# TorbenHellriegel/Speaker-Recognition-x-vectors

Measured on AMD Instinct MI355X. Metric: x-vector embeddings/sec (300-frame utt), higher is better.
Workload: dtype f32; 1 GPU; configs[1]: 1xMI355X batch=256 fixed 300-frame x 24-MFCC utterances, fp32 frame-level stack, extract_x_vec layer 6, random-init weights seed 42; build=xvec_hip gfx950 build df48636768b7, batch_per_gpu=256, frames=300

## Files before the change

### speaker-recognition-x-vectors_amd/csrc/tdnn_common.h

```cpp
#pragma once
#include "xvec_internal.h"

namespace xvec {

typedef float f32x16 __attribute__((ext_vector_type(16)));
typedef unsigned int u32x4 __attribute__((ext_vector_type(4)));
typedef float f32x4 __attribute__((ext_vector_type(4)));
typedef __bf16 bf16x8 __attribute__((ext_vector_type(8)));

#define SB() __builtin_amdgcn_sched_barrier(0)

__device__ __forceinline__ int xcd_remap(int bid, int nwg) {
    const int q = nwg >> 3, r = nwg & 7, xcd = bid & 7, local = bid >> 3;
    const int base = (xcd < r) ? xcd * (q + 1) : r * (q + 1) + (xcd - r) * q;
    return base + local;
}

typedef float f32x2 __attribute__((ext_vector_type(2)));
typedef __bf16 bf16x2 __attribute__((ext_vector_type(2)));

__device__ __forceinline__ float add_halves(float x) {
    const unsigned u = __float_as_uint(x);
    const auto r = __builtin_amdgcn_permlane32_swap(u, u, false, false);
    return __uint_as_float(r[0]) + __uint_as_float(r[1]);
}

__device__ __forceinline__ unsigned long long uniform64(unsigned long long v) {
    const unsigned lo = __builtin_amdgcn_readfirstlane((unsigned)v);
    const unsigned hi = __builtin_amdgcn_readfirstlane((unsigned)(v >> 32));
    return ((unsigned long long)hi << 32) | lo;
}

__device__ __forceinline__ __amdgpu_buffer_rsrc_t make_rsrc_n(const void* p, int num_bytes) {
    void* q = reinterpret_cast<void*>(uniform64(reinterpret_cast<unsigned long long>(p)));
    return __builtin_amdgcn_make_buffer_rsrc(q, (short)0, __builtin_amdgcn_readfirstlane(num_bytes), 0x00020000);
}

__device__ __forceinline__ __amdgpu_buffer_rsrc_t make_rsrc(const void* p) { return make_rsrc_n(p, 0x7fffffff); }

__device__ __forceinline__ __amdgpu_buffer_rsrc_t make_rsrc_bounded(const void* base, int64_t off, int64_t total) {
    int64_t left = total - off;
    left = left < 0 ? 0 : (left > 0x7fffffff ? 0x7fffffff : left);
    return make_rsrc_n(static_cast<const char*>(base) + off, (int)left);
}

__device__ __forceinline__ float4 buf_load16(__amdgpu_buffer_rsrc_t rsrc, int voff, int soff) {
    const u32x4 v = __builtin_amdgcn_raw_buffer_load_b128(rsrc, voff, soff, 0);
    const f32x4 f = __builtin_bit_cast(f32x4, v);
    return make_float4(f.x, f.y, f.z, f.w);
}

__device__ __forceinline__ void group_range(const TdnnArgs& a, int p, int64_t& begin, int64_t& end) {
    int64_t g_begin, g_end;
    if (a.pair_period > 0) {
        const int P = a.blocks_per_col, PQ = a.pair_period, hq = PQ >> 1;
        const int64_t base = a.groups_total / P;
        const int rem = (int)(a.groups_total % P);
        const int rem1 = rem < (P >> 1) ? rem : (P >> 1), rem2 = rem - rem1;
        const int xq = p / PQ, w = p % PQ;
        const int nf = xq * hq + (w < hq ? w : hq);
        const int ns = xq * hq + (w > hq ? w - hq : 0);
        g_begin = base * p + (nf < rem1 ? nf : rem1) + (ns < rem2 ? ns : rem2);
        const bool extra = (w < hq) ? (nf < rem1) : (ns < rem2);
        g_end = g_begin + base + (extra ? 1 : 0);
    } else {
        g_begin = a.groups_total * (int64_t)p / a.blocks_per_col;
        g_end = a.groups_total * (int64_t)(p + 1) / a.blocks_per_col;
    }
    begin = g_begin;
    end = g_end;
}

__host__ __device__ __forceinline__ int wino_pair_count(int T, int d) {
    const int r = T % (2 * d);
    return d * (T / (2 * d)) + (r < d ? r : d);
}

typedef unsigned u32x2 __attribute__((ext_vector_type(2)));

__device__ __forceinline__ void split3(const float4& v, u32x2& hi, u32x2& mid, u32x2& lo) {
    typedef __bf16 bf16x4v __attribute__((ext_vector_type(4)));
    const f32x4 x = {v.x, v.y, v.z, v.w};
    const bf16x4v h = __builtin_convertvector(x, bf16x4v);
    const f32x4 r1 = x - __builtin_convertvector(h, f32x4);
    const bf16x4v m = __builtin_convertvector(r1, bf16x4v);
    const f32x4 r2 = r1 - __builtin_convertvector(m, f32x4);
    const bf16x4v l = __builtin_convertvector(r2, bf16x4v);
    hi = __builtin_bit_cast(u32x2, h);
    mid = __builtin_bit_cast(u32x2, m);
    lo = __builtin_bit_cast(u32x2, l);
}

__device__ __forceinline__ void s3_mfma6(f32x16& acc, const float4* x, const float4* w) {
#define XV_S3M(xp_, wp_) \
    acc = __builtin_amdgcn_mfma_f32_32x32x16_bf16(__builtin_bit_cast(bf16x8, x[xp_]), __builtin_bit_cast(bf16x8, w[wp_]), acc, 0, 0, 0);
    XV_S3M(2, 0) XV_S3M(1, 1) XV_S3M(0, 2) XV_S3M(1, 0) XV_S3M(0, 1) XV_S3M(0, 0)
#undef XV_S3M
}

__device__ __forceinline__ void store_acc(const f32x16& v, const float4 (&sc)[4], const float4 (&sh)[4],
                                          __amdgpu_buffer_rsrc_t yrsrc, int y_voff, int y_soff) {
    unsigned pk[8];
    typedef float f32x2v __attribute__((ext_vector_type(2)));
#pragma unroll
    for (int gq = 0; gq < 4; ++gq) {
        const float y0 = fmaf(fmaxf(v[4 * gq + 0], 0.f), sc[gq].x, sh[gq].x);
        const float y1 = fmaf(fmaxf(v[4 * gq + 1], 0.f), sc[gq].y, sh[gq].y);
        const float y2 = fmaf(fmaxf(v[4 * gq + 2], 0.f), sc[gq].z, sh[gq].z);
        const float y3 = fmaf(fmaxf(v[4 * gq + 3], 0.f), sc[gq].w, sh[gq].w);
        pk[2 * gq] = __builtin_bit_cast(unsigned, __builtin_convertvector(f32x2v{y0, y1}, bf16x2));
        pk[2 * gq + 1] = __builtin_bit_cast(unsigned, __builtin_convertvector(f32x2v{y2, y3}, bf16x2));
    }
#pragma unroll
    for (int pr = 0; pr < 2; ++pr) {
        auto r0 = __builtin_amdgcn_permlane32_swap(pk[4 * pr + 0], pk[4 * pr + 2], false, false);
        auto r1 = __builtin_amdgcn_permlane32_swap(pk[4 * pr + 1], pk[4 * pr + 3], false, false);
        const u32x4 o = {r0[0], r1[0], r0[1], r1[1]};
        __builtin_amdgcn_raw_buffer_store_b128(o, yrsrc, y_voff, y_soff + pr * 32, 0);
        asm volatile("s_nop 1" ::"v"(o));
    }
}

__device__ __forceinline__ float lower_half(float x) {
    const unsigned u = __float_as_uint(x);
    const auto r = __builtin_amdgcn_permlane32_swap(u, u, false, false);
    return __uint_as_float(r[0]);
}

constexpr int kPoolPlanes = 3;

__device__ __forceinline__ void store_partial(__amdgpu_buffer_rsrc_t prs, int ld, int64_t slot, int h, int col, float k,
                                              float v0, float v1) {
    const int soff = (int)(slot * kPoolPlanes * ld) * 4;
    __builtin_amdgcn_raw_buffer_store_b32(__float_as_uint(h ? v1 : v0), prs, (col + (1 + h) * ld) * 4, soff, 0);
    if (h == 0) __builtin_amdgcn_raw_buffer_store_b32(__float_as_uint(k), prs, col * 4, soff, 0);
}

__device__ __forceinline__ void store_partial2(__amdgpu_buffer_rsrc_t prs, int ld, int64_t slot, int h, int col, float ka,
                                               float kb, float s1a, float s2a, float s1b, float s2b) {
    typedef unsigned u32x2 __attribute__((ext_vector_type(2)));
    const int soff = (int)(slot * kPoolPlanes * ld) * 4;
    const u32x2 v = {__float_as_uint(h ? s2a : s1a), __float_as_uint(h ? s2b : s1b)};
    __builtin_amdgcn_raw_buffer_store_b64(v, prs, (col + (1 + h) * ld) * 4, soff, 0);
    if (h == 0) {
        const u32x2 kv = {__float_as_uint(ka), __float_as_uint(kb)};
        __builtin_amdgcn_raw_buffer_store_b64(kv, prs, col * 4, soff, 0);
    }
}

struct PoolCur {
    int u;
    int64_t end;
};

__device__ __forceinline__ int64_t sload_i64(const int64_t* p) {
    int64_t v;
    asm volatile("s_load_dwordx2 %0, %1, 0x0\n\ts_waitcnt lgkmcnt(0)" : "=s"(v) : "s"(p) : "memory");
    return v;
}

template <bool RAGGED>
__device__ __forceinline__ int64_t first_row(const RowMap& m, int u) {
    u = __builtin_amdgcn_readfirstlane(u);
    if (RAGGED) return sload_i64(m.offsets + u) - (int64_t)u * m.cum;
    return (int64_t)u * (m.fixed_T - m.cum);
}

__device__ __forceinline__ float max1(float x, float m) {
    float r;
    asm("v_max_f32 %0, %1, %2" : "=v"(r) : "v"(x), "v"(m));
    return r;
}

template <bool RAGGED>
__device__ __forceinline__ void pool_group_impl(const TdnnArgs& a, const f32x16& v, float negk, int64_t row_g, int h,
                                                int col, PoolCur& pc) {
    const int64_t grp = row_g >> 5;
    const RowMap& m = a.out_map;
    const __amdgpu_buffer_rsrc_t prs = make_rsrc(a.pool_part);
    while (pc.end <= row_g && pc.u < m.n_utts - 1) {
        pc.u = __builtin_amdgcn_readfirstlane(pc.u + 1);
        pc.end = first_row<RAGGED>(m, pc.u + 1);
    }
    const float K = -negk;
    if (pc.end >= row_g + 32) {
        float a0 = max1(v[0], negk), a1 = max1(v[1], negk), a2 = max1(v[2], negk), a3 = max1(v[3], negk);
        float b0 = a0 * a0, b1 = a1 * a1, b2 = a2 * a2, b3 = a3 * a3;
#pragma unroll
        for (int e = 4; e < 16; e += 4) {
            const float d0 = max1(v[e], negk), d1 = max1(v[e + 1], negk), d2 = max1(v[e + 2], negk), d3 = max1(v[e + 3], negk);
            a0 += d0; a1 += d1; a2 += d2; a3 += d3;
            b0 = fmaf(d0, d0, b0); b1 = fmaf(d1, d1, b1); b2 = fmaf(d2, d2, b2); b3 = fmaf(d3, d3, b3);
        }
        const float s1 = add_halves((a0 + a1) + (a2 + a3)), s2 = add_halves((b0 + b1) + (b2 + b3));
        store_partial(prs, a.ldy, grp + pc.u, h, col, K, s1, s2);
        return;
    }
    for (int u = pc.u; u < m.n_utts; u = __builtin_amdgcn_readfirstlane(u + 1)) {
        const int64_t off = first_row<RAGGED>(m, u);
        if (off >= row_g + 32) break;
        const int64_t end = first_row<RAGGED>(m, u + 1);
        const int64_t lo_r = off > row_g ? off : row_g;
        const int64_t hi_r = end < row_g + 32 ? end : row_g + 32;
        if (hi_r <= lo_r) continue;
        const int lo_l = (int)(lo_r - row_g), hi_l = (int)(hi_r - row_g);
        const unsigned below_hi = hi_l >= 32 ? 0xffffffffu : ((1u << hi_l) - 1u);
        const unsigned rowmask = below_hi & ~((1u << lo_l) - 1u);
        const unsigned lm = rowmask >> (4 * h);
        float s1 = 0.f, s2 = 0.f;
#pragma unroll
        for (int e = 0; e < 16; ++e) {
            const float d = ((lm >> ((e & 3) + 8 * (e >> 2))) & 1u) ? max1(v[e], negk) : 0.f;
            s1 += d;
            s2 = fmaf(d, d, s2);
        }
        s1 = add_halves(s1);
        s2 = add_halves(s2);
        store_partial(prs, a.ldy, grp + u, h, col, K, s1, s2);
    }
}

__device__ __forceinline__ void pool_group(const TdnnArgs& a, const f32x16& v, float negk, int64_t row_g, int h, int col,
                                           PoolCur& pc) {
    if (a.out_map.offsets == nullptr) pool_group_impl<false>(a, v, negk, row_g, h, col, pc);
    else pool_group_impl<true>(a, v, negk, row_g, h, col, pc);
}

__device__ __forceinline__ PoolCur pool_cursor(const TdnnArgs& a, int64_t row) {
    PoolCur pc;
    pc.u = __builtin_amdgcn_readfirstlane(utt_of_row(a.out_map, row));
    pc.end = row_off(a.out_map, pc.u + 1);
    return pc;
}

}
```

### speaker-recognition-x-vectors_amd/csrc/tdnn_layer_impl.h

```cpp
#pragma once
#include <cstdlib>

#include "tdnn_common.h"

namespace xvec {

constexpr int kBM = 128, kBN = 128;
constexpr int kStageFloats = (kBM + kBN) * kBK;
constexpr int kConstFloats = 3 * kBN;
constexpr int kLdsBytes = (2 * kStageFloats + kConstFloats) * 4;

#ifdef XVEC_DIAG
static __device__ unsigned long long g_diag[8 * 8192];
#endif

struct Ctx {
    __amdgpu_buffer_rsrc_t xrsrc;
    __amdgpu_buffer_rsrc_t wrsrc;
    int x_base;
    int ur0, ur1, ur2, ur3;
    int xo0, xo1, xo2, xo3;
    int w_toff;
    __amdgpu_buffer_rsrc_t wfrsrc;
    int wf_voff;
    int r0;
    int u_tile;
    int64_t off_next;
    int64_t m0;
    int64_t g_s, g_end;
    PoolCur pool;
    bool pivot_set;
    int tap, kc, itl;
    int es;
};

__device__ __forceinline__ float4 cvt8_bf16(const float4& lo, const float4& hi) {
    typedef __bf16 bf16x8v __attribute__((ext_vector_type(8)));
    typedef float f32x8v __attribute__((ext_vector_type(8)));
    const f32x8v f8 = {lo.x, lo.y, lo.z, lo.w, hi.x, hi.y, hi.z, hi.w};
    const f32x4 b4 = __builtin_bit_cast(f32x4, __builtin_convertvector(f8, bf16x8v));
    return make_float4(b4.x, b4.y, b4.z, b4.w);
}

template <bool RAGGED>
__device__ __forceinline__ void set_tile_rows_impl(const TdnnArgs& a, Ctx& cx) {
    const int n_last = a.out_map.n_utts - 1;
    const int64_t t_out = a.out_map.fixed_T - a.out_map.cum;
    auto next_off = [&](int u) -> int64_t {
        if (RAGGED) return a.out_map.offsets[u + 1] - (int64_t)(u + 1) * a.out_map.cum;
        return (int64_t)(u + 1) * t_out;
    };
    while (cx.m0 >= cx.off_next && cx.u_tile < n_last) {
        cx.u_tile = __builtin_amdgcn_readfirstlane(cx.u_tile + 1);
        cx.off_next = next_off(cx.u_tile);
    }
    const int64_t p = cx.m0 + cx.r0;
    int c0 = 0, c1 = 0, c2 = 0, c3 = 0;
    int u = cx.u_tile;
    int64_t nxt = cx.off_next;
    while (nxt < cx.m0 + 128 && u < n_last) {
        c0 += (p >= nxt) ? 1 : 0;
        c1 += (p + 32 >= nxt) ? 1 : 0;
        c2 += (p + 64 >= nxt) ? 1 : 0;
        c3 += (p + 96 >= nxt) ? 1 : 0;
        u = __builtin_amdgcn_readfirstlane(u + 1);
        nxt = next_off(u);
    }
    const int rb = a.ldx * cx.es;
    cx.ur0 = (cx.u_tile + c0) * a.span;
    cx.ur1 = (cx.u_tile + c1) * a.span;
    cx.ur2 = (cx.u_tile + c2) * a.span;
    cx.ur3 = (cx.u_tile + c3) * a.span;
    cx.xo0 = cx.x_base + cx.ur0 * rb;
    cx.xo1 = cx.x_base + cx.ur1 * rb;
    cx.xo2 = cx.x_base + cx.ur2 * rb;
    cx.xo3 = cx.x_base + cx.ur3 * rb;
}

__device__ __forceinline__ void set_tile_rows(const TdnnArgs& a, Ctx& cx) {
    if (a.span == 0) {
        cx.ur0 = cx.ur1 = cx.ur2 = cx.ur3 = 0;
        cx.xo0 = cx.xo1 = cx.xo2 = cx.xo3 = cx.x_base;
        return;
    }
    if (a.out_map.offsets == nullptr) set_tile_rows_impl<false>(a, cx);
    else set_tile_rows_impl<true>(a, cx);
}

template <int GUARD>
__device__ __forceinline__ __amdgpu_buffer_rsrc_t x_rsrc(const TdnnArgs& a, const Ctx& cx) {
    const int src_es = GUARD == 2 ? 4 : cx.es;
    const int64_t off = cx.m0 * (int64_t)a.ldx * src_es;
    if (GUARD) return make_rsrc_bounded(a.X, off, a.x_bytes ? a.x_bytes : a.x_rows * (int64_t)a.ldx * src_es);
    return make_rsrc(static_cast<const char*>(a.X) + off);
}

template <int GUARD, bool X3>
__device__ __forceinline__ void advance(const TdnnArgs& a, Ctx& cx, int n_chunks) {
    if (cx.itl + 1 < n_chunks) {
        ++cx.itl;
        if (++cx.tap == a.n_taps) {
            cx.tap = 0;
            ++cx.kc;
        }
    } else {
        const int64_t g_rem = cx.g_end - cx.g_s;
        const int64_t g_next = cx.g_s + (g_rem < 4 ? g_rem : 4);
        if (g_next < cx.g_end) {
            cx.g_s = g_next;
            cx.m0 = g_next * 32;
            cx.xrsrc = x_rsrc<GUARD>(a, cx);
            set_tile_rows(a, cx);
            cx.itl = 0;
            cx.kc = 0;
            cx.tap = 0;
        }
    }
}

#define XV_KO(q_) ((((2 * (q_)) + h) ^ sw) << 2)
#define XV_FRG_A(i_, q_, f_, S_) \
    if constexpr (G > i_) { rg.fa##i_##_##f_ = *reinterpret_cast<const float4*>((S_) + a_rd + i_ * 32 * kBK + XV_KO(q_)); }
#define XV_FRG_B(q_, f_, S_) \
    if constexpr (!INBF) { rg.fb_##f_ = *reinterpret_cast<const float4*>((S_) + b_rd + XV_KO(q_)); }
#define XV_LST_A(i_, n_) \
    if constexpr (G > i_) { *reinterpret_cast<float4*>(smem + n_ * kStageFloats + st_off + i_ * 32 * kBK) = rg.sA##i_##_##n_; }
#define XV_LST_B(j_, n_)                                                                                  \
    if constexpr (X3) {                                                                                   \
        if constexpr (G > j_) *reinterpret_cast<float4*>(smem + n_ * kStageFloats + st_off + kBM * kBK + j_ * 32 * kBK) = rg.sB##j_##_##n_; \
    } else if constexpr (!INBF) {                                                                         \
        *reinterpret_cast<float4*>(smem + n_ * kStageFloats + st_off + kBM * kBK + j_ * 32 * kBK) = rg.sB##j_##_##n_; \
    }
#define XV_LST3(i_, b_)                                                                                   \
    if constexpr (G > i_) {                                                                               \
        *reinterpret_cast<float4*>(smem + b_ * kStageFloats + st_off + i_ * 32 * kBK) = rg.sA##i_##_0;      \
        *reinterpret_cast<float4*>(smem + b_ * kStageFloats + st_off + kBM * kBK + i_ * 32 * kBK) = rg.sB##i_##_0; \
    }
#define XV_GLD_X(dst_, i_, P_OFF)                                                                         \
    {                                                                                                     \
        const int row_shift = cx.tap * a.tap_rows;                                                        \
        const int soff = ((row_shift + 32 * i_) * a.ldx + cx.kc * BKE) * ES + (P_OFF);                    \
        if (GUARD) {                                                                                      \
                  \
            const bool ok_ = cx.kc * BKE + c * (16 / ES) < a.kpt;                                         \
            if constexpr (GUARD == 2) {                              \
                const int voff = ok_ ? 2 * cx.xo##i_ : 0x7ffffff0;                                        \
                const float4 lo_ = buf_load16(cx.xrsrc, voff, 2 * soff);                                  \
                const float4 hi_ = buf_load16(cx.xrsrc, voff, 2 * soff + 16);                             \
                dst_ = cvt8_bf16(lo_, hi_);                                                               \
            } else {                                                                                      \
                const int voff = ok_ ? cx.xo##i_ : 0x7ffffff0;                                            \
                dst_ = buf_load16(cx.xrsrc, voff, soff);                                                  \
            }                                                                                             \
        } else {                                                                                          \
            dst_ = buf_load16(cx.xrsrc, cx.xo##i_, soff);                                                 \
        }                                                                                                 \
    }
#define XV_GLD_A(i_, n_) \
    if constexpr (G > i_) XV_GLD_X(rg.sA##i_##_##n_, i_, 0)
#define XV_GLD_B(j_, n_)                                                                                  \
    if constexpr (X3) {                                                                                   \
        if constexpr (G > j_) XV_GLD_X(rg.sB##j_##_##n_, j_, a.x_plane_bytes)                             \
    } else if constexpr (!INBF) {                                                                         \
        rg.sB##j_##_##n_ = buf_load16(cx.wrsrc, cx.w_toff, (32 * j_ * a.k_pad + cx.itl * BKE) * ES);         \
    }
#define XV_GLB(q_, s_, c_)                                                                                \
    if constexpr (INBF && !X3) {                                                                          \
        int cw_ = (c_);                                                                                   \
        if (cw_ >= n_chunks) cw_ -= n_chunks;                                                             \
        rg.gb##q_##_##s_ = buf_load16(cx.wfrsrc, cx.wf_voff, (4 * cw_ + q_) * 1024);                      \
    }
#define XV_GLB3(q_, c_)                                                                                   \
    if constexpr (X3) {                                                                                   \
        int cw_ = (c_);                                                                                   \
        if (cw_ >= n_chunks) cw_ -= n_chunks;                                                             \
        rg.gb##q_##_0 = buf_load16(cx.wfrsrc, cx.wf_voff, (8 * cw_ + q_) * 1024);                         \
        rg.gb##q_##_1 = buf_load16(cx.wfrsrc, cx.wf_voff, (8 * cw_ + 4 + q_) * 1024);                     \
    }
#define XV_FRG_L(i_, q_, S_) \
    if constexpr (G > i_) { rg.fa##i_##_1 = *reinterpret_cast<const float4*>((S_) + kBM * kBK + a_rd + i_ * 32 * kBK + XV_KO(q_)); }
#define XV_GLD_ALL(n_) XV_GLD_A(0, n_) XV_GLD_A(1, n_) XV_GLD_A(2, n_) XV_GLD_A(3, n_) \
                       XV_GLD_B(0, n_) XV_GLD_B(1, n_) XV_GLD_B(2, n_) XV_GLD_B(3, n_)
#define XV_LST_ALL(n_) XV_LST_A(0, n_) XV_LST_A(1, n_) XV_LST_A(2, n_) XV_LST_A(3, n_) \
                       XV_LST_B(0, n_) XV_LST_B(1, n_) XV_LST_B(2, n_) XV_LST_B(3, n_)
#define XV_MF(i_, c_, f_, slot_)                                                                          \
    if constexpr (G > i_) {                                                                               \
        acc##i_ = __builtin_amdgcn_mfma_f32_32x32x2f32(rg.fa##i_##_##f_.c_, rg.fb_##f_.c_, acc##i_, 0, 0, 0);   \
    }                                                                                                     \
    SB();                                                                                                 \
    slot_                                                                                                 \
    SB();
#define XV_MFB(i_, f_, q_, P_)                                                                            \
    if constexpr (G > i_) {                                                                               \
        if constexpr (SWAP)                                                                               \
            acc##i_ = __builtin_amdgcn_mfma_f32_32x32x16_bf16(__builtin_bit_cast(bf16x8, rg.gb##q_##_##P_), \
                                                              __builtin_bit_cast(bf16x8, rg.fa##i_##_##f_), acc##i_, 0, 0, 0); \
        else                                                                                              \
            acc##i_ = __builtin_amdgcn_mfma_f32_32x32x16_bf16(__builtin_bit_cast(bf16x8, rg.fa##i_##_##f_), \
                                                              __builtin_bit_cast(bf16x8, rg.gb##q_##_##P_), acc##i_, 0, 0, 0); \
    }                                                                                                     \
    SB();
#define XV_KG(q_, P_, f_, s0, s1, s2, s3, s4, s5, s6, s7, s8, s9, s10, s11, s12, s13, s14, s15)           \
    if constexpr (INBF) {                                                                                 \
        XV_MFB(0, f_, q_, P_) s0 s1 s2 s3 SB(); XV_MFB(1, f_, q_, P_) s4 s5 s6 s7 SB();                   \
        XV_MFB(2, f_, q_, P_) s8 s9 s10 s11 SB(); XV_MFB(3, f_, q_, P_) s12 s13 s14 s15 SB();             \
    } else {                                                                                              \
        XV_MF(0, x, f_, s0) XV_MF(1, x, f_, s1) XV_MF(2, x, f_, s2) XV_MF(3, x, f_, s3)                   \
        XV_MF(0, y, f_, s4) XV_MF(1, y, f_, s5) XV_MF(2, y, f_, s6) XV_MF(3, y, f_, s7)                   \
        XV_MF(0, z, f_, s8) XV_MF(1, z, f_, s9) XV_MF(2, z, f_, s10) XV_MF(3, z, f_, s11)                 \
        XV_MF(0, w, f_, s12) XV_MF(1, w, f_, s13) XV_MF(2, w, f_, s14) XV_MF(3, w, f_, s15)               \
    }
#define XV_M3(i_, f_, b_)                                                                                 \
    if constexpr (G > i_) {                                                                               \
        acc##i_ = __builtin_amdgcn_mfma_f32_32x32x16_bf16(__builtin_bit_cast(bf16x8, rg.fa##i_##_##f_),   \
                                                          __builtin_bit_cast(bf16x8, rg.b_), acc##i_, 0, 0, 0); \
    }                                                                                                     \
    SB();
#define XV_G3(f_, b_, s0, s1, s2, s3) \
    XV_M3(0, f_, b_) s0 SB(); XV_M3(1, f_, b_) s1 SB(); XV_M3(2, f_, b_) s2 SB(); XV_M3(3, f_, b_) s3 SB();
#define XV_NOP ;
#define XV_ADVANCE (advance<GUARD, X3>)(a, cx, n_chunks);
#define XV_CHUNK(P_, N_, IT_)                                                                             \
    {                                                                                                     \
        const float* S = smem + P_ * kStageFloats;                                                        \
        const float* Sn = smem + N_ * kStageFloats;                                                       \
        XV_KG(0, P_, 0, XV_FRG_A(0, 1, 1, S), XV_FRG_A(1, 1, 1, S), XV_FRG_A(2, 1, 1, S),                 \
              XV_FRG_A(3, 1, 1, S), XV_FRG_B(1, 1, S),                                                    \
              XV_LST_A(0, N_), XV_LST_A(1, N_), XV_LST_A(2, N_), XV_LST_A(3, N_),                         \
              XV_LST_B(0, N_), XV_LST_B(1, N_), XV_LST_B(2, N_), XV_LST_B(3, N_),                         \
              XV_GLB(3, N_, (IT_) + 1), XV_NOP, XV_ADVANCE)                                \
        XV_KG(1, P_, 1, XV_FRG_A(0, 2, 0, S), XV_FRG_A(1, 2, 0, S), XV_FRG_A(2, 2, 0, S),                 \
              XV_FRG_A(3, 2, 0, S), XV_FRG_B(2, 0, S),                                                    \
              XV_GLD_A(0, N_), XV_GLD_A(1, N_), XV_GLD_A(2, N_), XV_GLD_A(3, N_),                         \
              XV_GLD_B(0, N_), XV_GLD_B(1, N_), XV_GLD_B(2, N_), XV_GLD_B(3, N_),                         \
              XV_GLB(0, P_, (IT_) + 2), XV_NOP, XV_NOP)                                                   \
        XV_KG(2, P_, 0, XV_FRG_A(0, 3, 1, S), XV_FRG_A(1, 3, 1, S), XV_FRG_A(2, 3, 1, S),                 \
              XV_FRG_A(3, 3, 1, S), XV_FRG_B(3, 1, S), XV_GLB(1, P_, (IT_) + 2), XV_NOP, XV_NOP, XV_NOP,  \
              XV_NOP, XV_NOP, XV_NOP, XV_NOP, XV_NOP, XV_NOP, XV_NOP)                                     \
        __syncthreads();                      \
        XV_KG(3, P_, 1, XV_FRG_A(0, 0, 0, Sn), XV_FRG_A(1, 0, 0, Sn), XV_FRG_A(2, 0, 0, Sn),              \
              XV_FRG_A(3, 0, 0, Sn), XV_FRG_B(0, 0, Sn), XV_GLB(2, P_, (IT_) + 2), XV_NOP, XV_NOP,        \
              XV_NOP, XV_NOP, XV_NOP, XV_NOP, XV_NOP, XV_NOP, XV_NOP, XV_NOP)                             \
    }

#define XV_CHUNK3(P_, N_, IT_)                                                                            \
    {                                                                                                     \
        const float* S = smem + P_ * kStageFloats;                                                        \
        const float* Sn = smem + N_ * kStageFloats;                                                       \
        XV_G3(0, gb0_0, XV_FRG_L(0, 0, S), XV_FRG_L(1, 0, S), XV_FRG_L(2, 0, S), XV_FRG_L(3, 0, S))       \
        XV_G3(0, gb0_1, XV_LST3(0, N_), XV_LST3(1, N_), XV_LST3(2, N_), XV_LST3(3, N_))                   \
        XV_G3(1, gb0_0, XV_FRG_A(0, 1, 0, S), XV_FRG_A(1, 1, 0, S), XV_FRG_A(2, 1, 0, S),                 \
              XV_FRG_A(3, 1, 0, S))                                                                       \
        XV_ADVANCE                                                                                        \
        XV_G3(0, gb1_0, XV_FRG_L(0, 1, S), XV_FRG_L(1, 1, S), XV_FRG_L(2, 1, S), XV_FRG_L(3, 1, S))       \
        XV_G3(0, gb1_1, XV_GLB3(0, (IT_) + 1), XV_GLD_A(0, 0) XV_GLD_A(1, 0),                             \
              XV_GLD_A(2, 0) XV_GLD_A(3, 0), XV_GLD_B(0, 0) XV_GLD_B(1, 0))                               \
        XV_G3(1, gb1_0, XV_FRG_A(0, 2, 0, S), XV_FRG_A(1, 2, 0, S), XV_FRG_A(2, 2, 0, S),                 \
              XV_FRG_A(3, 2, 0, S))                                                                       \
        XV_G3(0, gb2_0, XV_FRG_L(0, 2, S), XV_FRG_L(1, 2, S), XV_FRG_L(2, 2, S), XV_FRG_L(3, 2, S))       \
        XV_G3(0, gb2_1, XV_GLB3(1, (IT_) + 1), XV_GLD_B(2, 0) XV_GLD_B(3, 0), XV_NOP, XV_NOP)             \
        XV_G3(1, gb2_0, XV_FRG_A(0, 3, 0, S), XV_FRG_A(1, 3, 0, S), XV_FRG_A(2, 3, 0, S),                 \
              XV_FRG_A(3, 3, 0, S))                                                                       \
        XV_G3(0, gb3_0, XV_FRG_L(0, 3, S), XV_FRG_L(1, 3, S), XV_FRG_L(2, 3, S), XV_FRG_L(3, 3, S))       \
        XV_G3(0, gb3_1, XV_GLB3(2, (IT_) + 1), XV_NOP, XV_NOP, XV_NOP)                                    \
        __syncthreads();                      \
        XV_G3(1, gb3_0, XV_FRG_A(0, 0, 0, Sn), XV_FRG_A(1, 0, 0, Sn), XV_FRG_A(2, 0, 0, Sn),              \
              XV_FRG_A(3, 0, 0, Sn))                                                                      \
        XV_GLB3(3, (IT_) + 1)                                                                             \
    }

struct Regs {
    float4 sA0_0, sA1_0, sA2_0, sA3_0, sB0_0, sB1_0, sB2_0, sB3_0;
    float4 sA0_1, sA1_1, sA2_1, sA3_1, sB0_1, sB1_1, sB2_1, sB3_1;
    float4 fa0_0, fa1_0, fa2_0, fa3_0, fb_0, fa0_1, fa1_1, fa2_1, fa3_1, fb_1;
    float4 gb0_0, gb1_0, gb2_0, gb3_0, gb0_1, gb1_1, gb2_1, gb3_1;
    float4 w3[2][6];
};

struct Lane {
    int h, sw, a_rd, b_rd, st_off, r0, c, col;
    int st3, rd3;
};

constexpr int kPlaneBytes = kBM * kBK * 2;

__device__ __forceinline__ void s3_store(char* B, int st3, int i, const float4& v) {
    u32x2 hi, mid, lo;
    split3(v, hi, mid, lo);
    *reinterpret_cast<u32x2*>(B + st3 + i * 32 * 64) = hi;
    *reinterpret_cast<u32x2*>(B + kPlaneBytes + st3 + i * 32 * 64) = mid;
    *reinterpret_cast<u32x2*>(B + 2 * kPlaneBytes + st3 + i * 32 * 64) = lo;
}

template <int NG>
__device__ __forceinline__ void s3_gld(const TdnnArgs& a, const Ctx& cx, float4& d0, float4& d1, float4& d2, float4& d3) {
    const int soff = ((cx.tap * a.tap_rows) * a.ldx + cx.kc * kBK) * 4;
    const int rs = 32 * a.ldx * 4;
    if constexpr (NG > 0) d0 = buf_load16(cx.xrsrc, cx.xo0, soff);
    if constexpr (NG > 1) d1 = buf_load16(cx.xrsrc, cx.xo1, soff + rs);
    if constexpr (NG > 2) d2 = buf_load16(cx.xrsrc, cx.xo2, soff + 2 * rs);
    if constexpr (NG > 3) d3 = buf_load16(cx.xrsrc, cx.xo3, soff + 3 * rs);
}

__device__ __forceinline__ void s3_wld(const Ctx& cx, float4* w, int c, int n_chunks) {
    if (c >= n_chunks) c -= n_chunks;
#pragma unroll
    for (int j = 0; j < 6; ++j) w[j] = buf_load16(cx.wfrsrc, cx.wf_voff, (6 * c + j) * 1024);
}

#define XV_S3_CHUNK(P_, N_, IT_)                                                                          \
    {                                                                                                     \
        const char* S = reinterpret_cast<const char*>(smem) + P_ * kStageFloats * 4;                      \
        char* Sn = reinterpret_cast<char*>(smem) + N_ * kStageFloats * 4;                                 \
        if constexpr (G > 0) s3_store(Sn, ln.st3, 0, rg.sA0_##N_);                                         \
        if constexpr (G > 1) s3_store(Sn, ln.st3, 1, rg.sA1_##N_);                                         \
        if constexpr (G > 2) s3_store(Sn, ln.st3, 2, rg.sA2_##N_);                                         \
        if constexpr (G > 3) s3_store(Sn, ln.st3, 3, rg.sA3_##N_);                                         \
        advance<GUARD, false>(a, cx, n_chunks);                                                           \
        s3_gld<G>(a, cx, rg.sA0_##N_, rg.sA1_##N_, rg.sA2_##N_, rg.sA3_##N_);                              \
        s3_wld(cx, rg.w3[N_], (IT_) + 1, n_chunks);                                                       \
        _Pragma("unroll") for (int s3 = 0; s3 < 2; ++s3) {                                                \
            const int rd = ln.rd3 ^ (32 * s3);                                                            \
            float4 xf[4][3];                                                                              \
            _Pragma("unroll") for (int i = 0; i < G; ++i)                                                 \
                _Pragma("unroll") for (int pl = 0; pl < 3; ++pl)                                          \
                    xf[i][pl] = *reinterpret_cast<const float4*>(S + pl * kPlaneBytes + i * 32 * 64 + rd); \
            if constexpr (G > 0) s3_mfma6(acc0, xf[0], rg.w3[P_] + 3 * s3);                                \
            if constexpr (G > 1) s3_mfma6(acc1, xf[1], rg.w3[P_] + 3 * s3);                                \
            if constexpr (G > 2) s3_mfma6(acc2, xf[2], rg.w3[P_] + 3 * s3);                                \
            if constexpr (G > 3) s3_mfma6(acc3, xf[3], rg.w3[P_] + 3 * s3);                                \
        }                                                                                                 \
        __syncthreads();                      \
    }

template <int GUARD, bool INBF, bool X3, bool S3>
__device__ __forceinline__ void block_prologue(const TdnnArgs& a, float* smem, Ctx& cx, Regs& rg, const Lane& ln,
                                               int n_chunks) {
    constexpr int G = 4;
    constexpr int ES = INBF ? 2 : 4, BKE = 128 / ES;
    const int h = ln.h, sw = ln.sw, a_rd = ln.a_rd, b_rd = ln.b_rd, st_off = ln.st_off, c = ln.c;
    if constexpr (S3) {
        char* B0 = reinterpret_cast<char*>(smem);
        s3_gld<4>(a, cx, rg.sA0_0, rg.sA1_0, rg.sA2_0, rg.sA3_0);
        advance<GUARD, false>(a, cx, n_chunks);
        s3_gld<4>(a, cx, rg.sA0_1, rg.sA1_1, rg.sA2_1, rg.sA3_1);
        s3_wld(cx, rg.w3[0], 0, n_chunks);
        s3_store(B0, ln.st3, 0, rg.sA0_0);
        s3_store(B0, ln.st3, 1, rg.sA1_0);
        s3_store(B0, ln.st3, 2, rg.sA2_0);
        s3_store(B0, ln.st3, 3, rg.sA3_0);
        advance<GUARD, false>(a, cx, n_chunks);
        s3_gld<4>(a, cx, rg.sA0_0, rg.sA1_0, rg.sA2_0, rg.sA3_0);
        __syncthreads();
        return;
    }
    if constexpr (X3) {
        XV_GLD_ALL(0)
        SB();
        XV_LST3(0, 0) XV_LST3(1, 0) XV_LST3(2, 0) XV_LST3(3, 0)
        SB();
        advance<GUARD, X3>(a, cx, n_chunks);
        XV_GLD_ALL(0)
    } else {
        XV_GLD_ALL(0)
        advance<GUARD, X3>(a, cx, n_chunks);
        XV_GLD_ALL(1)
        SB();
        XV_LST_ALL(0)
        SB();
        advance<GUARD, X3>(a, cx, n_chunks);
        XV_GLD_ALL(0)
    }
    __syncthreads();
    XV_FRG_A(0, 0, 0, smem) XV_FRG_A(1, 0, 0, smem) XV_FRG_A(2, 0, 0, smem) XV_FRG_A(3, 0, 0, smem)
    XV_FRG_B(0, 0, smem)
    XV_GLB(0, 0, 0) XV_GLB(1, 0, 0) XV_GLB(2, 0, 0) XV_GLB(3, 0, 0)
    XV_GLB(0, 1, 1) XV_GLB(1, 1, 1) XV_GLB(2, 1, 1) XV_GLB(3, 1, 1)
    XV_GLB3(0, 0) XV_GLB3(1, 0) XV_GLB3(2, 0) XV_GLB3(3, 0)
    SB();
}

template <int G, int GUARD, bool POOL, bool STORE, bool INBF, bool OUTBF, bool X3, bool S3>
__device__ __forceinline__ void process_tile(const TdnnArgs& a, float* smem, Ctx& cx, Regs& rg, const Lane& ln,
                                             int64_t g0, int n0, int n_chunks) {
    constexpr int ES = INBF ? 2 : 4, BKE = 128 / ES;
    const int h = ln.h, sw = ln.sw, a_rd = ln.a_rd, b_rd = ln.b_rd, st_off = ln.st_off, c = ln.c;
    constexpr bool SWAP = INBF && OUTBF && !X3 && STORE && !POOL;
    f32x16 acc0, acc1, acc2, acc3;
    const float* cstw = smem + 2 * kStageFloats + (ln.col - n0 - (int)(threadIdx.x & 31)) + 4 * ln.h;
    if constexpr (SWAP) {
#pragma unroll
        for (int gq = 0; gq < 4; ++gq) {
            const float4 b4 = *reinterpret_cast<const float4*>(cstw + 8 * gq);
            acc0[4 * gq] = b4.x; acc0[4 * gq + 1] = b4.y; acc0[4 * gq + 2] = b4.z; acc0[4 * gq + 3] = b4.w;
        }
        acc1 = acc0; acc2 = acc0; acc3 = acc0;
    } else if constexpr (POOL) {
        const float b0 = smem[2 * kStageFloats + kBN + (ln.col - n0)];
#pragma unroll
        for (int e = 0; e < 16; ++e) acc0[e] = b0;
        acc1 = acc0; acc2 = acc0; acc3 = acc0;
    } else {
#pragma unroll
        for (int e = 0; e < 16; ++e) { acc0[e] = 0.f; acc1[e] = 0.f; acc2[e] = 0.f; acc3[e] = 0.f; }
    }

#ifdef XVEC_DIAG
    SB();
    const unsigned long long dt0 = __builtin_amdgcn_s_memtime();
    SB();
#endif
    for (int it = 0; it < n_chunks; it += 2) {
        if constexpr (S3) {
            XV_S3_CHUNK(0, 1, it)
            XV_S3_CHUNK(1, 0, it + 1)
        } else if constexpr (X3) {
            XV_CHUNK3(0, 1, it)
            XV_CHUNK3(1, 0, it + 1)
        } else {
            XV_CHUNK(0, 1, it)
            XV_CHUNK(1, 0, it + 1)
        }
    }
#ifdef XVEC_DIAG
    SB();
    const unsigned long long dt1 = __builtin_amdgcn_s_memtime();
    SB();
#endif

    const int64_t m0 = g0 * 32;
    const int col = ln.col;
    float* cst = smem + 2 * kStageFloats + (col - n0);
    const float bi = cst[0], sc = cst[kBN], sh = cst[2 * kBN];
    float negk = sh;
    if constexpr (POOL) {
        if (!cx.pivot_set) {
            const float piv = lower_half(fmaxf(acc0[0] + bi, 0.f));
            const float bmk = bi - piv;
            negk = bmk - bi;
#pragma unroll
            for (int e = 0; e < 16; ++e) {
                acc0[e] += bmk;
                if constexpr (G > 1) acc1[e] += bmk;
                if constexpr (G > 2) acc2[e] += bmk;
                if constexpr (G > 3) acc3[e] += bmk;
            }
            cst[kBN] = bmk;
            cst[2 * kBN] = negk;
            cx.pivot_set = true;
        }
    }
    const int esz = OUTBF ? 2 : 4;
    __amdgpu_buffer_rsrc_t yrsrc;
    int y_voff = 0;
    __amdgpu_buffer_rsrc_t yrsrc_lo;
    if (STORE) {
        yrsrc = make_rsrc(static_cast<char*>(a.Y) + (m0 * (int64_t)a.ldy + n0) * esz);
        if constexpr (X3 && OUTBF)
            yrsrc_lo = make_rsrc(static_cast<char*>(a.Y) + a.y_plane_bytes + (m0 * (int64_t)a.ldy + n0) * esz);
        y_voff = (4 * h * a.ldy + (col - n0)) * esz;
    }
#define XV_EPI(i_)                                                                                        \
    if constexpr (G > i_) {                                                                               \
                                                                                       \
        if constexpr (!POOL) {                                                                            \
            _Pragma("unroll") for (int e = 0; e < 16; ++e)                                                \
                acc##i_[e] = fmaf(fmaxf(acc##i_[e] + bi, 0.f), sc, sh);                                   \
            asm volatile("" : "+v"(acc##i_));                                                             \
        }                                                                                                 \
        if (STORE) {                                                                                      \
            _Pragma("unroll") for (int e = 0; e < 16; ++e) {                                              \
                const int soff = (i_ * 32 + (e & 3) + 8 * (e >> 2)) * a.ldy * esz;                        \
                if constexpr (OUTBF) {                                                                    \
                    const __bf16 hv = (__bf16)acc##i_[e];                                                 \
                    __builtin_amdgcn_raw_buffer_store_b16(__builtin_bit_cast(unsigned short, hv), yrsrc,  \
                                                          y_voff, soff, 0);                               \
                    if constexpr (X3) {                   \
                        const __bf16 lv = (__bf16)(acc##i_[e] - (float)hv);                               \
                        __builtin_amdgcn_raw_buffer_store_b16(__builtin_bit_cast(unsigned short, lv),     \
                                                              yrsrc_lo, y_voff, soff, 0);                 \
                    }                                                                                     \
                } else {                                                                                  \
                    const float fv = acc##i_[e];  \
                    __builtin_amdgcn_raw_buffer_store_b32(__float_as_uint(fv), yrsrc, y_voff, soff, 0);   \
                }                                                                                         \
            }                                                                                             \
        }                                                                                                 \
        if (POOL) pool_group(a, acc##i_, negk, m0 + i_ * 32, h, col, cx.pool);                            \
    }
    if constexpr (SWAP) {
        float4 sc4[4], sh4[4];
#pragma unroll
        for (int gq = 0; gq < 4; ++gq) {
            sc4[gq] = *reinterpret_cast<const float4*>(cstw + kBN + 8 * gq);
            sh4[gq] = *reinterpret_cast<const float4*>(cstw + 2 * kBN + 8 * gq);
        }
        const int voff = ((int)(threadIdx.x & 31) * a.ldy + (ln.col - n0 - (int)(threadIdx.x & 31)) + 8 * h) * 2;
        if constexpr (G > 0) store_acc(acc0, sc4, sh4, yrsrc, voff, 0 * 32 * a.ldy * 2);
        if constexpr (G > 1) store_acc(acc1, sc4, sh4, yrsrc, voff, 1 * 32 * a.ldy * 2);
        if constexpr (G > 2) store_acc(acc2, sc4, sh4, yrsrc, voff, 2 * 32 * a.ldy * 2);
        if constexpr (G > 3) store_acc(acc3, sc4, sh4, yrsrc, voff, 3 * 32 * a.ldy * 2);
    } else {
        XV_EPI(0) XV_EPI(1) XV_EPI(2) XV_EPI(3)
    }
#undef XV_EPI
#ifdef XVEC_DIAG
    SB();
    asm volatile("s_waitcnt lgkmcnt(0)" ::: "memory");
    const unsigned long long dt2 = __builtin_amdgcn_s_memtime();
    SB();
    if (threadIdx.x == 0 && blockIdx.x < 8192) {
        unsigned long long* d = g_diag + blockIdx.x * 8;
        d[3] += dt1 - dt0;
        d[4] += dt2 - dt1;
        d[5] += 1;
    }
#endif
}

template <int GUARD, bool POOL, bool STORE, bool INBF, bool OUTBF, bool X3, bool S3>
__device__ __forceinline__ void tdnn_body(const TdnnArgs& a, float* smem) {
#ifdef XVEC_DIAG
    const unsigned long long t_entry = __builtin_amdgcn_s_memtime(), r_entry = __builtin_amdgcn_s_memrealtime();
    if (threadIdx.x == 0 && blockIdx.x < 8192) { g_diag[blockIdx.x * 8 + 3] = 0; g_diag[blockIdx.x * 8 + 4] = 0; g_diag[blockIdx.x * 8 + 5] = 0; }
#endif
    const int lid = xcd_remap(blockIdx.x, gridDim.x);
    const int j = lid % a.n_tiles;
    const int p = lid / a.n_tiles;
    int64_t g_begin, g_end;
    group_range(a, p, g_begin, g_end);
    const int n0 = j * kBN;
    const int n_chunks = a.n_taps * a.cpt;

    const int tid = threadIdx.x;
    const int lane = tid & 63, wave = tid >> 6;
    Lane ln;
    ln.h = lane >> 5;
    const int r = lane & 31;
    ln.c = tid & 7;
    ln.r0 = tid >> 3;
    ln.st_off = ln.r0 * kBK + ((ln.c ^ ((ln.r0 >> 1) & 7)) << 2);
    ln.sw = (r >> 1) & 7;
    ln.a_rd = r * kBK;
    ln.b_rd = kBM * kBK + (wave * 32 + r) * kBK;
    ln.col = n0 + wave * 32 + r;
    ln.st3 = ln.r0 * 64 + ((((ln.c >> 1) ^ ((ln.r0 >> 2) & 3)) * 16) | ((ln.c & 1) * 8));
    ln.rd3 = r * 64 + ((ln.h ^ ((r >> 2) & 3)) * 16);
    if (tid < kBN) {
        smem[2 * kStageFloats + tid] = a.bias[n0 + tid];
        smem[2 * kStageFloats + kBN + tid] = POOL ? 0.f : a.scale[n0 + tid];
        smem[2 * kStageFloats + 2 * kBN + tid] = POOL ? 0.f : a.shift[n0 + tid];
    }

    Ctx cx;
    cx.g_s = g_begin;
    cx.g_end = g_end;
    cx.m0 = g_begin * 32;
    constexpr int ES = INBF ? 2 : 4;
    cx.es = ES;
    cx.xrsrc = x_rsrc<GUARD>(a, cx);
    cx.wrsrc = make_rsrc(static_cast<const char*>(a.W) + (int64_t)n0 * a.k_pad * ES);
    cx.x_base = ln.r0 * a.ldx * ES + ln.c * 16;
    cx.w_toff = ln.r0 * a.k_pad * ES + ln.c * 16;
    cx.r0 = ln.r0;
    if (INBF) {
        const int64_t ct = n0 / 32 + wave;
        cx.wfrsrc = make_rsrc(static_cast<const char*>(a.Wf) + ct * (int64_t)(a.k_pad / 16) * 1024);
        cx.wf_voff = lane * 16;
    }
    if (S3) {
        const int64_t ct = n0 / 32 + wave;
        cx.wfrsrc = make_rsrc(static_cast<const char*>(a.Wf) + ct * (int64_t)(a.k_pad / 16) * 3072);
        cx.wf_voff = lane * 16;
    }
    cx.u_tile = __builtin_amdgcn_readfirstlane(utt_of_row(a.out_map, cx.m0));
    cx.off_next = row_off(a.out_map, cx.u_tile + 1);
    if (POOL) {
        cx.pool.u = cx.u_tile;
        cx.pool.end = cx.off_next;
    }
    cx.pivot_set = false;
    set_tile_rows(a, cx);
    cx.tap = 0;
    cx.kc = 0;
    cx.itl = 0;

    Regs rg;
    block_prologue<GUARD, INBF, X3, S3>(a, smem, cx, rg, ln, n_chunks);
    int64_t g = g_begin;
    for (; g + 4 <= g_end; g += 4) process_tile<4, GUARD, POOL, STORE, INBF, OUTBF, X3, S3>(a, smem, cx, rg, ln, g, n0, n_chunks);
    const int rem = (int)(g_end - g);
    if (rem == 3) process_tile<3, GUARD, POOL, STORE, INBF, OUTBF, X3, S3>(a, smem, cx, rg, ln, g, n0, n_chunks);
    else if (rem == 2) process_tile<2, GUARD, POOL, STORE, INBF, OUTBF, X3, S3>(a, smem, cx, rg, ln, g, n0, n_chunks);
    else if (rem == 1) process_tile<1, GUARD, POOL, STORE, INBF, OUTBF, X3, S3>(a, smem, cx, rg, ln, g, n0, n_chunks);
#ifdef XVEC_DIAG
    if (threadIdx.x == 0 && blockIdx.x < 8192) {
        __builtin_amdgcn_s_waitcnt(0);
        unsigned long long* d = g_diag + blockIdx.x * 8;
        d[0] = t_entry;
        d[1] = __builtin_amdgcn_s_memtime();
        d[2] = (unsigned long long)(g_end - g_begin);
        d[6] = r_entry;
        d[7] = __builtin_amdgcn_s_memrealtime();
    }
#endif
}

template <typename K>
static hipError_t launch_kernel(K kern, const TdnnArgs& a, hipStream_t s, LdsOptIn& opt) {
    if (a.groups_total <= 0 || a.blocks_per_col <= 0 || a.blocks_per_col > a.groups_total || (a.cpt & 1))
        return hipErrorInvalidValue;
    if (hipError_t e = opt.ensure(reinterpret_cast<const void*>(kern), kLdsBytes); e != hipSuccess) return e;
    const int grid = a.blocks_per_col * a.n_tiles;
    kern<<<dim3(grid), dim3(256), kLdsBytes, s>>>(a);
    return hipGetLastError();
}

}
```

Baseline: 147,200 embeddings/s.

## Interleave split3 conversion, LDS stores and prefetch reads into the S3 MFMA stream

Rewrites the split-bf16 (S3) chunk loop as a hand-scheduled software pipeline. The hi/mid/lo split of the next chunk's activations, their LDS stores and the next global loads are broken into eight small steps and spread across the 48 MFMAs, with sched barriers fencing each slot. LDS fragment reads are double-buffered in named registers one MFMA group ahead, and the barrier moves to just before the last group. The goal is to hide conversion, LDS and VMEM latency behind the matrix cores instead of running them as serial phases, at the cost of more live registers, possible occupancy loss, and fragile barrier and ordering logic.

```diff
diff --git a/speaker-recognition-x-vectors_amd/csrc/tdnn_common.h b/speaker-recognition-x-vectors_amd/csrc/tdnn_common.h
--- a/speaker-recognition-x-vectors_amd/csrc/tdnn_common.h
+++ b/speaker-recognition-x-vectors_amd/csrc/tdnn_common.h
@@ -91,6 +91,21 @@
     lo = __builtin_bit_cast(u32x2, l);
 }
 
+__device__ __forceinline__ u32x2 s3_piece(const f32x4& r) {
+    typedef __bf16 bf16x4v __attribute__((ext_vector_type(4)));
+    return __builtin_bit_cast(u32x2, __builtin_convertvector(r, bf16x4v));
+}
+__device__ __forceinline__ void s3_rem_lo(f32x4& r, const u32x2& p) {
+    const unsigned w = p.x;
+    r.x -= __uint_as_float(w << 16);
+    r.y -= __uint_as_float(w & 0xffff0000u);
+}
+__device__ __forceinline__ void s3_rem_hi(f32x4& r, const u32x2& p) {
+    const unsigned w = p.y;
+    r.z -= __uint_as_float(w << 16);
+    r.w -= __uint_as_float(w & 0xffff0000u);
+}
+
 __device__ __forceinline__ void s3_mfma6(f32x16& acc, const float4* x, const float4* w) {
 #define XV_S3M(xp_, wp_) \
     acc = __builtin_amdgcn_mfma_f32_32x32x16_bf16(__builtin_bit_cast(bf16x8, x[xp_]), __builtin_bit_cast(bf16x8, w[wp_]), acc, 0, 0, 0);
diff --git a/speaker-recognition-x-vectors_amd/csrc/tdnn_layer_impl.h b/speaker-recognition-x-vectors_amd/csrc/tdnn_layer_impl.h
--- a/speaker-recognition-x-vectors_amd/csrc/tdnn_layer_impl.h
+++ b/speaker-recognition-x-vectors_amd/csrc/tdnn_layer_impl.h
@@ -274,7 +274,8 @@
     float4 sA0_1, sA1_1, sA2_1, sA3_1, sB0_1, sB1_1, sB2_1, sB3_1;
     float4 fa0_0, fa1_0, fa2_0, fa3_0, fb_0, fa0_1, fa1_1, fa2_1, fa3_1, fb_1;
     float4 gb0_0, gb1_0, gb2_0, gb3_0, gb0_1, gb1_1, gb2_1, gb3_1;
-    float4 w3[2][6];
+    float4 w0_0, w1_0, w2_0, w3_0, w4_0, w5_0, w0_1, w1_1, w2_1, w3_1, w4_1, w5_1;
+    float4 xf0_0, xf0_1, xf0_2, xf1_0, xf1_1, xf1_2;
 };
 
 struct Lane {
@@ -302,35 +303,108 @@
     if constexpr (NG > 3) d3 = buf_load16(cx.xrsrc, cx.xo3, soff + 3 * rs);
 }
 
-__device__ __forceinline__ void s3_wld(const Ctx& cx, float4* w, int c, int n_chunks) {
-    if (c >= n_chunks) c -= n_chunks;
-#pragma unroll
-    for (int j = 0; j < 6; ++j) w[j] = buf_load16(cx.wfrsrc, cx.wf_voff, (6 * c + j) * 1024);
-}
+#define XV_S3_WLD(n_, c_)                                                                                 \
+    {                                                                                                     \
+        int cw_ = (c_);                                                                                   \
+        if (cw_ >= n_chunks) cw_ -= n_chunks;                                                             \
+        rg.w0_##n_ = buf_load16(cx.wfrsrc, cx.wf_voff, (6 * cw_ + 0) * 1024);                             \
+        rg.w1_##n_ = buf_load16(cx.wfrsrc, cx.wf_voff, (6 * cw_ + 1) * 1024);                             \
+        rg.w2_##n_ = buf_load16(cx.wfrsrc, cx.wf_voff, (6 * cw_ + 2) * 1024);                             \
+        rg.w3_##n_ = buf_load16(cx.wfrsrc, cx.wf_voff, (6 * cw_ + 3) * 1024);                             \
+        rg.w4_##n_ = buf_load16(cx.wfrsrc, cx.wf_voff, (6 * cw_ + 4) * 1024);                             \
+        rg.w5_##n_ = buf_load16(cx.wfrsrc, cx.wf_voff, (6 * cw_ + 5) * 1024);                             \
+    }
+
+constexpr int s3_slot_of(int q, int G) { return q * (12 * G - 6) / (8 * G); }
+constexpr int s3_step_in(int n, int G, int k) {
+    int found = 0;
+    for (int q = 0; q < 8 * G; ++q) {
+        if (s3_slot_of(q, G) != n) continue;
+        if (found == k) return q;
+        ++found;
+    }
+    return -1;
+}
+#define XV_S3_ST(pl_, i_) *reinterpret_cast<u32x2*>(Sn + pl_ * kPlaneBytes + ln.st3 + i_ * 32 * 64) = sp;
+#define XV_S3_STEP(i_, N_, st_)                                                                           \
+    if constexpr (st_ == 0) {                                                                             \
+        sr = f32x4{rg.sA##i_##_##N_.x, rg.sA##i_##_##N_.y, rg.sA##i_##_##N_.z, rg.sA##i_##_##N_.w};       \
+        sp = s3_piece(sr);                                                                        \
+    } else if constexpr (st_ == 1) {                                                                      \
+        s3_rem_lo(sr, sp);                                                                                \
+    } else if constexpr (st_ == 2) {                                                                      \
+        s3_rem_hi(sr, sp);                                                                                \
+    } else if constexpr (st_ == 3) {                                                                      \
+        XV_S3_ST(0, i_)                                                                                   \
+        rg.sA##i_##_##N_ = buf_load16(cx.xrsrc, cx.xo##i_, g_soff + i_ * g_rs);                           \
+    } else if constexpr (st_ == 4) {                                                                      \
+        sp = s3_piece(sr);                                                                       \
+    } else if constexpr (st_ == 5) {                                                                      \
+        XV_S3_ST(1, i_)                                                                                   \
+        s3_rem_lo(sr, sp);                                                                                \
+    } else if constexpr (st_ == 6) {                                                                      \
+        s3_rem_hi(sr, sp);                                                                                \
+    } else {                                                                                              \
+        sp = s3_piece(sr);                                                                        \
+        XV_S3_ST(2, i_)                                                                                   \
+    }
+#define XV_S3_STEPQ(q_, N_)                                                                               \
+    {                                                                                                     \
+        constexpr int sq_ = (q_);                                                                         \
+        if constexpr (sq_ >= 0) {                                                                         \
+            constexpr int st_ = sq_ & 7;                                                                  \
+            if constexpr ((sq_ >> 3) == 0) { XV_S3_STEP(0, N_, st_) }                                     \
+            else if constexpr ((sq_ >> 3) == 1) { XV_S3_STEP(1, N_, st_) }                                \
+            else if constexpr ((sq_ >> 3) == 2) { XV_S3_STEP(2, N_, st_) }                                \
+            else { XV_S3_STEP(3, N_, st_) }                                                               \
+        }                                                                                                 \
+    }
+#define XV_S3_RD(s_, i_, XN_, pl_)                                                                        \
+    {                                                                                                     \
+        constexpr int ni_ = (i_ + 1 < G) ? i_ + 1 : 0, ns_ = (i_ + 1 < G) ? s_ : s_ + 1;                  \
+        rg.xf##XN_##_##pl_ = *reinterpret_cast<const float4*>((ns_ < 2 ? S : Sn) + pl_ * kPlaneBytes + ni_ * 32 * 64 + \
+                                                              (ns_ == 1 ? rd1 : rd0));                    \
+    }
+#define XV_S3_M(s_, i_, XS_, XN_, xp_, wj_, P_, N_, j_)                                                   \
+    acc##i_ = __builtin_amdgcn_mfma_f32_32x32x16_bf16(__builtin_bit_cast(bf16x8, rg.xf##XS_##_##xp_),     \
+                                                      __builtin_bit_cast(bf16x8, rg.w##wj_##_##P_), acc##i_, 0, 0, 0); \
+    SB();                                                                                                 \
+    if constexpr (j_ == 0) XV_S3_RD(s_, i_, XN_, 0)                                                       \
+    if constexpr (j_ == 1) XV_S3_RD(s_, i_, XN_, 1)                                                       \
+    if constexpr (j_ == 2) XV_S3_RD(s_, i_, XN_, 2)                                                       \
+    XV_S3_STEPQ(s3_step_in(6 * (s_ * G + i_) + j_, G, 0), N_)                                             \
+    XV_S3_STEPQ(s3_step_in(6 * (s_ * G + i_) + j_, G, 1), N_)                                             \
+    SB();
+#define XV_S3_G6(s_, i_, XS_, XN_, WH_, WM_, WL_, P_, N_)                                                 \
+    XV_S3_M(s_, i_, XS_, XN_, 2, WH_, P_, N_, 0) XV_S3_M(s_, i_, XS_, XN_, 1, WM_, P_, N_, 1)             \
+    XV_S3_M(s_, i_, XS_, XN_, 0, WL_, P_, N_, 2) XV_S3_M(s_, i_, XS_, XN_, 1, WH_, P_, N_, 3)             \
+    XV_S3_M(s_, i_, XS_, XN_, 0, WM_, P_, N_, 4) XV_S3_M(s_, i_, XS_, XN_, 0, WH_, P_, N_, 5)
+#define XV_S3_GRP(s_, i_, WH_, WM_, WL_, P_, N_)                                                          \
+    if constexpr (G > i_) {                                                                               \
+        if constexpr (s_ == 1 && i_ == G - 1) {                                                           \
+            __syncthreads();                              \
+            SB();                                                                                         \
+        }                                                                                                 \
+        if constexpr (((s_ * G + i_) & 1) == 0) { XV_S3_G6(s_, i_, 0, 1, WH_, WM_, WL_, P_, N_) }         \
+        else { XV_S3_G6(s_, i_, 1, 0, WH_, WM_, WL_, P_, N_) }                                            \
+    }
 
 #define XV_S3_CHUNK(P_, N_, IT_)                                                                          \
     {                                                                                                     \
         const char* S = reinterpret_cast<const char*>(smem) + P_ * kStageFloats * 4;                      \
         char* Sn = reinterpret_cast<char*>(smem) + N_ * kStageFloats * 4;                                 \
-        if constexpr (G > 0) s3_store(Sn, ln.st3, 0, rg.sA0_##N_);                                         \
-        if constexpr (G > 1) s3_store(Sn, ln.st3, 1, rg.sA1_##N_);                                         \
-        if constexpr (G > 2) s3_store(Sn, ln.st3, 2, rg.sA2_##N_);                                         \
-        if constexpr (G > 3) s3_store(Sn, ln.st3, 3, rg.sA3_##N_);                                         \
         advance<GUARD, false>(a, cx, n_chunks);                                                           \
-        s3_gld<G>(a, cx, rg.sA0_##N_, rg.sA1_##N_, rg.sA2_##N_, rg.sA3_##N_);                              \
-        s3_wld(cx, rg.w3[N_], (IT_) + 1, n_chunks);                                                       \
-        _Pragma("unroll") for (int s3 = 0; s3 < 2; ++s3) {                                                \
-            const int rd = ln.rd3 ^ (32 * s3);                                                            \
-            float4 xf[4][3];                                                                              \
-            _Pragma("unroll") for (int i = 0; i < G; ++i)                                                 \
-                _Pragma("unroll") for (int pl = 0; pl < 3; ++pl)                                          \
-                    xf[i][pl] = *reinterpret_cast<const float4*>(S + pl * kPlaneBytes + i * 32 * 64 + rd); \
-            if constexpr (G > 0) s3_mfma6(acc0, xf[0], rg.w3[P_] + 3 * s3);                                \
-            if constexpr (G > 1) s3_mfma6(acc1, xf[1], rg.w3[P_] + 3 * s3);                                \
-            if constexpr (G > 2) s3_mfma6(acc2, xf[2], rg.w3[P_] + 3 * s3);                                \
-            if constexpr (G > 3) s3_mfma6(acc3, xf[3], rg.w3[P_] + 3 * s3);                                \
-        }                                                                                                 \
-        __syncthreads();                      \
+        const int g_soff = ((cx.tap * a.tap_rows) * a.ldx + cx.kc * kBK) * 4, g_rs = 32 * a.ldx * 4;      \
+        const int rd0 = ln.rd3, rd1 = ln.rd3 ^ 32;                    \
+        f32x4 sr;                                                                                         \
+        u32x2 sp;                                                                                         \
+        SB();                                                                                             \
+        XV_S3_WLD(N_, (IT_) + 1)                                                                          \
+        SB();                                                                                             \
+        XV_S3_GRP(0, 0, 0, 1, 2, P_, N_) XV_S3_GRP(0, 1, 0, 1, 2, P_, N_)                                 \
+        XV_S3_GRP(0, 2, 0, 1, 2, P_, N_) XV_S3_GRP(0, 3, 0, 1, 2, P_, N_)                                 \
+        XV_S3_GRP(1, 0, 3, 4, 5, P_, N_) XV_S3_GRP(1, 1, 3, 4, 5, P_, N_)                                 \
+        XV_S3_GRP(1, 2, 3, 4, 5, P_, N_) XV_S3_GRP(1, 3, 3, 4, 5, P_, N_)                                 \
     }
 
 template <int GUARD, bool INBF, bool X3, bool S3>
@@ -344,7 +418,7 @@
         s3_gld<4>(a, cx, rg.sA0_0, rg.sA1_0, rg.sA2_0, rg.sA3_0);
         advance<GUARD, false>(a, cx, n_chunks);
         s3_gld<4>(a, cx, rg.sA0_1, rg.sA1_1, rg.sA2_1, rg.sA3_1);
-        s3_wld(cx, rg.w3[0], 0, n_chunks);
+        XV_S3_WLD(0, 0)
         s3_store(B0, ln.st3, 0, rg.sA0_0);
         s3_store(B0, ln.st3, 1, rg.sA1_0);
         s3_store(B0, ln.st3, 2, rg.sA2_0);
@@ -352,6 +426,9 @@
         advance<GUARD, false>(a, cx, n_chunks);
         s3_gld<4>(a, cx, rg.sA0_0, rg.sA1_0, rg.sA2_0, rg.sA3_0);
         __syncthreads();
+        rg.xf0_0 = *reinterpret_cast<const float4*>(B0 + ln.rd3);
+        rg.xf0_1 = *reinterpret_cast<const float4*>(B0 + kPlaneBytes + ln.rd3);
+        rg.xf0_2 = *reinterpret_cast<const float4*>(B0 + 2 * kPlaneBytes + ln.rd3);
         return;
     }
     if constexpr (X3) {
```

Result: faster. 152,400 embeddings/s (median of 6 runs) (+3.5%).
